# datatypevoid/babble

Measured on AMD Instinct MI355X. Metric: consensus-ordered events/sec at N=256 peers (1 GPU and 8-GPU batched sims), higher is better.
Workload: dtype int32

## Files before the change

babble_amd/csrc/hgx_api.cpp:

```cpp
#include <algorithm>
#include <array>
#include <chrono>
#include <cstdio>
#include <cstring>
#include <mutex>
#include <tuple>
#include <set>
#include <new>
#include <cstdlib>
#include <string>
#include <thread>
#include <vector>

#include "hgx.h"
#include "hgx_bodies.h"
#include "hgx_bodystore.h"
#include "hgx_diff.h"
#include "hgx_engine.h"
#include "hgx_wire_plan.h"

namespace {

struct Block {
    int32_t rr;
// ... 2736 lines not shown
    DeviceGuard dg(c);
    if (ensure_mirror(c) || !same_graph(c, x, y)) return 0;
    std::vector<int32_t> lx(c->n), fx(c->n), ly(c->n), fy(c->n);
    if (c->eng.get_coords(x, lx.data(), fx.data()) != hipSuccess) return 0;
    if (c->eng.get_coords(y, ly.data(), fy.data()) != hipSuccess) return 0;
    int cnt = 0;
    for (int i = 0; i < c->n; i++) cnt += lx[i] >= fy[i];
    return cnt >= c->sm ? 1 : 0;
}
int64_t hgx_oldest_self_ancestor_to_see(hgx_ctx* c, int64_t x, int64_t y) {
    if (!known_div(c, x) || !known_div(c, y)) return -1;
    DeviceGuard dg(c);
    if (ensure_chains(c) || !same_graph(c, x, y)) return -1;
    std::vector<int32_t> la(c->n), fd(c->n);
    if (c->eng.get_coords(y, la.data(), fd.data()) != hipSuccess) return -1;
    const int cx = c->creator[(size_t)x];
    const int32_t a = fd[cx % c->n];
    if (a <= c->index32[(size_t)x]) return c->chain_gids[cx][(size_t)(a - c->chain_base[cx])];
    return -1;
}
int32_t hgx_round(hgx_ctx* c, int64_t x) {
    if (!c) return -1;
    DeviceGuard dg(c);
    if (ensure_rounds(c)) return -1;
    return round_of(c, x);
}
int32_t hgx_witness(hgx_ctx* c, int64_t x) {
    if (!c) return 0;
    DeviceGuard dg(c);
    if (ensure_rounds(c) || ensure_mirror(c)) return 0;
    return witness_of(c, x);
}

int32_t hgx_phase_times(hgx_ctx* c, double* out, int32_t cap) {
    if (!c || !out) return 0;
    const int32_t m = std::min<int32_t>(cap, 28);
    double v[28] = {c->eng.phase_ms[0], c->eng.phase_ms[1], c->eng.phase_ms[2], c->eng.phase_ms[3],
                    (double)c->eng.la_sweeps, (double)c->eng.R, (double)c->eng.compact,
                    (double)c->eng.la_rows, c->eng.last_rebuild ? 1.0 : 0.0, (double)c->rh.r_lo,
                    c->eng.la_wave_used ? 1.0 : 0.0, (double)c->eng.la_wave_fallbacks,
                    (double)(c->eng.la_wave_used ? c->eng.la_wave_segs : 0), (double)c->eng.round_p_runs,
                    (double)c->eng.round_p_fallbacks, (double)c->eng.round_p_ovf,
                    (double)c->eng.round_p_fail_round, (double)c->eng.round_p_fail_chain,
                    (double)c->eng.round_g_runs, c->eng.la_small_used ? 1.0 : 0.0,
                    c->eng.la_verified ? 1.0 : 0.0, (double)c->eng.sort_seg_runs, (double)c->eng.pipe_used,
                    c->host_ms[0], c->host_ms[1], c->host_ms[2], c->host_ms[3], (double)c->eng.cts_row_runs};
    for (int32_t i = 0; i < m; i++) out[i] = v[i];
    return m;
}

static const char* kKernelNames[hgx::K_NUM] = {"layout", "la_sweep", "fd_build", "round_gather", "round_search",
                                              "fame", "threshold", "round_received", "cts_median", "order_sort"};

int32_t hgx_kernel_stats(hgx_ctx* c, int32_t k, char* name, int32_t name_cap, double* ms, int64_t* launches,
                         double* bytes) {
    if (!c || k < 0 || k >= hgx::K_NUM) return HGX_ERR_INVALID;
    if (name && name_cap > 0) std::snprintf(name, (size_t)name_cap, "%s", kKernelNames[k]);
    const hgx::KernelStat& ks = c->eng.kstat[k];
    if (ms) *ms = (ks.timed > 0 && ks.timed < ks.launches) ? ks.ms * (double)ks.launches / (double)ks.timed : ks.ms;
    if (launches) *launches = c->eng.kstat[k].launches;
    if (bytes) *bytes = c->eng.kstat[k].bytes;
    return HGX_OK;
}

int32_t hgx_reset_stats(hgx_ctx* c) {
    if (!c) return HGX_ERR_INVALID;
    for (auto& s : c->eng.kstat) s = hgx::KernelStat();
    return HGX_OK;
}

int32_t hgx_set_coord_storage(hgx_ctx* c, int32_t mode) {
    if (!c || mode < 0 || mode > 1) return HGX_ERR_INVALID;
    each_shard(c, [&](hgx_ctx* x) { x->eng.force_coord32 = mode == 1; });
    return HGX_OK;
}

int32_t hgx_set_kernel_timing(hgx_ctx* c, int32_t on) {
    if (!c) return HGX_ERR_INVALID;
    each_shard(c, [&](hgx_ctx* x) { x->eng.time_mask = (uint32_t)on; });
    return HGX_OK;
}

int32_t hgx_set_fame_tally(hgx_ctx* c, int32_t mode) {
    if (!c || mode < 0 || mode > 2) return HGX_ERR_INVALID;
    each_shard(c, [&](hgx_ctx* x) { x->eng.fame_tally = mode; });
    return HGX_OK;
}

int32_t hgx_device_alloc(int32_t device, int64_t bytes, void** ptr) {
    if (!ptr || bytes < 0) return HGX_ERR_INVALID;
    *ptr = nullptr;
    int prev = -1;
    (void)hipGetDevice(&prev);
    if (hipSetDevice(device) != hipSuccess) return HGX_ERR_DEVICE;
    const hipError_t e = hipMalloc(ptr, (size_t)std::max<int64_t>(bytes, 1));
    if (prev >= 0 && prev != device) (void)hipSetDevice(prev);
    return e == hipSuccess ? HGX_OK : HGX_ERR_DEVICE;
}

int32_t hgx_device_free(int32_t device, void* ptr) {
    int prev = -1;
    (void)hipGetDevice(&prev);
    if (hipSetDevice(device) != hipSuccess) return HGX_ERR_DEVICE;
    const hipError_t e = ptr ? hipFree(ptr) : hipSuccess;
    if (prev >= 0 && prev != device) (void)hipSetDevice(prev);
    return e == hipSuccess ? HGX_OK : HGX_ERR_DEVICE;
}

int32_t hgx_device_copy(int32_t device, void* dst, const void* src, int64_t bytes, int32_t to_device) {
    if (bytes < 0 || (bytes > 0 && (!dst || !src))) return HGX_ERR_INVALID;
    int prev = -1;
    (void)hipGetDevice(&prev);
    if (hipSetDevice(device) != hipSuccess) return HGX_ERR_DEVICE;
    const hipError_t e = bytes ? hipMemcpy(dst, src, (size_t)bytes, to_device ? hipMemcpyHostToDevice
                                                                               : hipMemcpyDeviceToHost)
                               : hipSuccess;
    if (prev >= 0 && prev != device) (void)hipSetDevice(prev);
    return e == hipSuccess ? HGX_OK : HGX_ERR_DEVICE;
}

int32_t hgx_set_ingest_pipeline(hgx_ctx* c, int32_t pieces, int64_t min_events) {
    if (!c || pieces < 0 || pieces > hgx::kPipeMaxPieces || min_events < 0) return HGX_ERR_INVALID;
    each_shard(c, [&](hgx_ctx* x) {
        x->eng.pipe_pieces = pieces;
        x->eng.pipe_min = min_events;
    });
    return HGX_OK;
}

int32_t hgx_set_la_kernel(hgx_ctx* c, int32_t mode) {
    if (!c || mode < 0 || mode > 1026) return HGX_ERR_INVALID;
    each_shard(c, [&](hgx_ctx* x) {
        x->eng.la_kernel = mode == 1 ? 1 : 0;
        x->eng.la_segs_override = (mode >= 2 && mode <= 1024) ? mode : 0;
        x->eng.la_small_override = mode == 1025 ? 0 : -1;
        x->eng.la_verify_always = mode == 1026;
    });
    return HGX_OK;
}

int32_t hgx_set_root_others(hgx_ctx* c, const uint8_t* event_hash32, int64_t count, hgx_error* err) {
    if (!c || count < 0 || (count > 0 && !event_hash32)) {
        set_err(err, HGX_ERR_INVALID, "hgx_set_root_others: bad arguments");
        return HGX_ERR_INVALID;
    }
    if (group_only_one(c, err, "hgx_set_root_others")) return HGX_ERR_INVALID;
    if (!c->rooted && count > 0) {
        set_err(err, HGX_ERR_INVALID, "hgx_set_root_others: no roots installed (hgx_reset)");
        return HGX_ERR_INVALID;
    }
    DeviceGuard dg(c);
    const hipError_t e = c->eng.set_root_others(event_hash32, count);
    if (e != hipSuccess) return dev_err(err, e, "hgx_set_root_others");
    c->others_keys.assign(event_hash32, event_hash32 + (size_t)count * 32);
    return ok(err);
}

int32_t hgx_set_sort_kernel(hgx_ctx* c, int32_t mode) {
    if (!c || mode < 0 || mode > 1) return HGX_ERR_INVALID;
    each_shard(c, [&](hgx_ctx* x) { x->eng.sort_seg_enabled = mode == 0; });
    return HGX_OK;
}

int32_t hgx_set_round_kernel(hgx_ctx* c, int32_t mode) {
    if (!c || mode < 0 || mode > 5) return HGX_ERR_INVALID;
    each_shard(c, [&](hgx_ctx* x) {
        x->eng.round_kernel = mode == 5 ? 0 : mode;
// ... 160 lines not shown
```

babble_amd/csrc/hgx_engine.cpp:

```cpp
#include "hgx_engine.h"
#include "hgx_bodystore.h"

#include <algorithm>
#include <array>
#include <chrono>
#include <cstdio>
#include <cstdlib>
#include <cstring>
#include <functional>

namespace hgx {

template <typename T>
hipError_t DBuf<T>::alloc(size_t count) {
    release();
    if (count == 0) count = 1;
    hipError_t e = hipMalloc((void**)&p, count * sizeof(T));
    if (e == hipSuccess) n = count; else p = nullptr;
    return e;
}

template <typename T>
hipError_t DBuf<T>::grow_copy(size_t count, size_t keep, hipStream_t s) {
    if (count <= n) return hipSuccess;
// ... 1291 lines not shown
    return hipStreamSynchronize(stream);
}

hipError_t Engine::get_event_fields(int64_t gid, int64_t* ts, int32_t* ntx, int32_t* tx_nil) {
    uint8_t nil = 0;
    HGX_TRY(hipMemcpyAsync(ts, g_ts.p + gid, 8, hipMemcpyDeviceToHost, stream));
    HGX_TRY(hipMemcpyAsync(ntx, g_ntx.p + gid, 4, hipMemcpyDeviceToHost, stream));
    HGX_TRY(hipMemcpyAsync(&nil, g_txnil.p + gid, 1, hipMemcpyDeviceToHost, stream));
    HGX_TRY(hipStreamSynchronize(stream));
    *tx_nil = nil;
    return hipSuccess;
}

hipError_t Engine::reserve_rounds(int32_t rounds) {
    rounds = std::max<int32_t>(rounds, 1);
    drop_step_graph();
    Bm.release(); WLA.release(); WFD.release(); wflag.release(); wstat.release(); wcoin.release();
    active.release(); Tthr.release(); fw.release(); elig.release(); ur_empty.release(); Smat.release();
    Vbuf.release(); fame.release(); blk_cnt.release(); blk_loaded.release(); blk_ntx.release(); blk_nil.release();
    ovf.release();
    WLAT.release();
    r_cap = 0;
    R = 0;
    E_div = 0;
    HGX_TRY(ensure_round_cap(rounds));
    return hipStreamSynchronize(stream);
}

int Engine::rebuild_segments(int64_t En, int coord_compact) const {
    if (G != 1 || En < (int64_t)kLaSegMinRows * C) return 1;
    const int cap_segs = (int)std::max<int64_t>(kLaMaxSegs, En / C / (2 * kLaHeadRows));
    return la_segs_override > 0 ? la_segs_override : la_wave_segments(n, coord_compact, num_cus, cap_segs);
}

void Engine::divide_rounds_rows(RoundsHost& out) {
    if (!rows_pending) return;
    rows_pending = false;
    for (size_t k = 0; k < rows_n && k < stage_out.size(); k++) {
        StagedD2H& d = stage_out[k];
        std::memcpy(d.dst, h_stage + d.off, d.bytes);
        d.bytes = 0;
    }
    out.bm.resize((size_t)(R + 1) * C);
    out.wflag.resize((size_t)R * C);
}

int32_t Engine::recv_round_lo(const RoundsHost& rh, int& max_unrecv) const {
    int32_t lo = R;
    max_unrecv = 0;
    if (E_div == 0 || rh.R == 0) return lo;
    for (int c = 0; c < C; c++) {
        const int32_t k = h_fu[c], len = h_len_div[c];
        if (k >= len) continue;
        max_unrecv = std::max(max_unrecv, len - k);
        int32_t a = 0, b = rh.R;
        while (a < b) {
            const int32_t mid = (a + b + 1) / 2;
            if (rh.bm[(size_t)mid * C + c] <= k) a = mid; else b = mid - 1;
        }
        lo = std::min(lo, a + 1);
    }
    return lo;
}

hipError_t Engine::decide_fame(int32_t r0, std::vector<int8_t>& fame_out) {
    HGX_TRY(decide_fame_launch(r0, fame_out));
    return fame_pending ? decide_fame_wait() : hipSuccess;
}

hipError_t Engine::decide_fame_launch(int32_t r0, std::vector<int8_t>& fame_out) {
    fame_pending = false;
    if (!rows_pending) {
        stage_out.clear();
        stage_used = 0;
    }
    pend.clear();
    if (fame_out.size() < (size_t)R * C) fame_out.resize((size_t)R * C, 0);
    r0 = std::max(r0, 0);
    if (R <= r0) return hipSuccess;
    DevArrays a = arrays();
    HGX_TRY(hipEventRecord(ph0, stream));
    HGX_TRY(hipGetLastError());
    kbeg(K_FAME);
    launch_fame(stream, a, r0, R, C, n, nw, sm, G, fame_tally);
    kend(K_FAME, 0);
    HGX_TRY(hipGetLastError());
    const size_t o = (size_t)r0 * C;
    HGX_TRY(stage_d2h(fame_out.data() + o, fame.p + o, fame_out.size() - o));
    HGX_TRY(stage_issue());
    HGX_TRY(hipEventRecord(ph1, stream));
    fame_pending = true;
    return hipSuccess;
}

hipError_t Engine::decide_fame_wait() {
    if (!fame_pending) {
        return hipStreamSynchronize(stream);
    }
    fame_pending = false;
    HGX_TRY(hipEventSynchronize(ph1));
    stage_flush();
    float ms = 0;
    HGX_TRY(hipEventElapsedTime(&ms, ph0, ph1));
    phase_ms[2] = ms;
    return collect_kernel_times();
}

hipError_t Engine::find_order(const std::vector<uint8_t>& el, const std::vector<uint8_t>& famous,
                              const std::vector<uint8_t>& ure, int32_t r0, int max_unrecv, OrderHost& out) {
    HGX_TRY(find_order_begin(el, famous, ure, r0, max_unrecv, out));
    return find_order_end(out, nullptr);
}

hipError_t Engine::find_order_begin(const std::vector<uint8_t>& el, const std::vector<uint8_t>& famous,
                                    const std::vector<uint8_t>& ure, int32_t r0, int max_unrecv, OrderHost& out) {
    stage_out.clear();
    pend.clear();
    stage_used = 0;
    out = OrderHost();
    fo_m = 0;
    fo_cnt.assign(C, 0);
    if (R == 0 || E_div == 0 || max_unrecv == 0 || r0 >= R) return hipSuccess;
    DevArrays a = arrays();
    HGX_TRY(hipEventRecord(ph0, stream));
    const size_t o = (size_t)r0 * C;
    HGX_TRY(stage_h2d(elig.p, el.data(), (size_t)G * R));
    HGX_TRY(stage_h2d(fw.p + o, famous.data() + o, (size_t)R * C - o));
    HGX_TRY(stage_h2d(ur_empty.p, ure.data(), (size_t)G));
    HGX_TRY(stage_issue());
    if (WLAT.n < (size_t)R * C * n) {
        const size_t want = (size_t)R * C * n + (size_t)C * n;
        const size_t first = WLAT.n ? 0 : std::min((size_t)r_cap * C * n, (size_t)1 << 28);
        HGX_TRY(WLAT.alloc(std::max(want, std::max(2 * WLAT.n, first))));
        a = arrays();
    }
    kbeg(K_THRESHOLD);
    launch_wla_transpose(stream, a, r0, R, G, C, n);
    launch_threshold(stream, a, r0, R, C, n);
    kend(K_THRESHOLD, 0);
    {
        FillRange fr[2] = {{counters.p + kCtRecv, 8, 0}, {rcnt.p, (uint32_t)((size_t)C * 4), 0}};
        launch_fill_many(stream, fr, 2);
        HGX_TRY(hipGetLastError());
    }
    kbeg(K_ROUND_RECEIVED);
    launch_round_received(stream, a, R, C, n, max_unrecv);
    kend(K_ROUND_RECEIVED, 0);
    HGX_TRY(copy_to_pinned(h_small + kHsRecv, counters.p + kCtRecv, 8));
    HGX_TRY(stage_d2h(fo_cnt.data(), rcnt.p, (size_t)C * 4));
    HGX_TRY(stage_issue());
    HGX_TRY(hipStreamSynchronize(stream));
    stage_flush();
    fo_m = h_small[kHsRecv];
    out.panic = h_small[kHsRecv + 1] != 0;
    out.m = fo_m;
    int max_cnt = 0, unrecv = 0;
    for (int c = 0; c < C; c++) unrecv += h_len_div[c] - h_fu[c];
    for (int c = shard_lo; c < shard_hi; c++) max_cnt = std::max(max_cnt, fo_cnt[c]);
    kadd_bytes(K_ROUND_RECEIVED, (double)unrecv * 16);
    if (out.panic || fo_m == 0) {
        fo_m = 0;
        return collect_kernel_times();
    }
    int64_t own = 0;
    for (int c = shard_lo; c < shard_hi; c++) own += fo_cnt[c];
    const int c_cnt = shard_hi - shard_lo;
    constexpr int kCtsRowMinTiles = 8;
// ... 259 lines not shown
```

babble_amd/csrc/hgx_kernels.h:

```cpp
#pragma once

#include <hip/hip_runtime.h>

#include <cstdint>
#include <functional>
#include <vector>

namespace hgx {

constexpr int32_t kMaxI32 = 2147483647;
constexpr int32_t kWlatNotFamous = -2147483647 - 1;
constexpr int kOpkBits = 21;

struct DevArrays {
    const int32_t *g_creator, *g_index, *g_op, *g_ntx;
    const int64_t* g_ts;
    const uint8_t *g_S, *g_coin, *g_loaded, *g_txnil;
    int32_t *g_rr, *g_pos;
    int64_t* g_ck;
    int64_t* g_cts;
    const int32_t *c_off, *c_len, *c_base;
    int32_t *p_gid, *p_chain, *p_op, *p_opu, *p_round, *p_rr;
    int32_t* p_opk;
    int64_t *p_ts, *p_cts;
// ... 84 lines not shown
hipError_t ensure_lds_limit(const void* f, size_t bytes);
hipError_t blocks_per_cu(const void* f, int T, size_t lds, int* out);

struct FillRange {
    void* p;
    uint32_t bytes;
    uint8_t value;
};
constexpr int kFillMax = 8;
void launch_fill_many(hipStream_t s, const FillRange* r, int count);
struct CopyRange {
    const void* src;
    void* dst;
    uint32_t bytes;
    int reset = -1;
};
constexpr int kCopyMax = 8;
void launch_copy_many(hipStream_t s, const CopyRange* r, int count);

int fd_tile_rows(int n, int compact);
void launch_layout(hipStream_t s, int64_t E0, int64_t E, const DevArrays& a, int C, int n, int seg,
                   const int32_t* gate = nullptr);
bool la_wave_ok(int n, int max_len, int n_active);
size_t la_small_bytes(int n, int compact, int64_t P);
hipError_t launch_la_small(hipStream_t s, const DevArrays& a, int G, int n, const int32_t* c_old, size_t lds,
                           int32_t* err);
int la_wave_blocks(int n, int compact);
int la_wave_segments(int n, int compact, int num_cus, int max_segs);
hipError_t launch_la_seg_check(hipStream_t s, const DevArrays& a, int n, int64_t E, int nts, int head, int32_t* tbl,
                               int32_t* flag);
struct LaSubset {
    int first = 0, count = 0;
    const int32_t* c_lim = nullptr;
    const int32_t* gate = nullptr;
};
hipError_t launch_la_wave(hipStream_t s, const DevArrays& a, int G, int n, const int32_t* c_old, int64_t E, int nts,
                          int head, int32_t* err, const int32_t* lmap = nullptr, int na = 0,
                          bool narrow = false, const LaSubset& sub = LaSubset());
void launch_la_sweep(hipStream_t s, const DevArrays& a, int C, int n, int max_len, int seg, int first, int32_t* chg,
                     int32_t stamp, int64_t* usum, int32_t* out, int32_t* out_next, const int32_t* c_old, int64_t u0);
void launch_fd_build(hipStream_t s, const DevArrays& a, int C, int n, int max_len, int64_t P, const int32_t* c_old,
                     int max_new, int d_lo = 0, int d_hi = -1);
void launch_init_new(hipStream_t s, const DevArrays& a, int64_t E0, int64_t m, int n, int64_t P);
void launch_round_gather(hipStream_t s, const DevArrays& a, int r, int C, int n, int64_t P);
void launch_wcoin(hipStream_t s, const DevArrays& a, int r0, int R, int C);
hipError_t launch_round_step(hipStream_t s, const RoundArgs& A, int r, int block_search);
hipError_t launch_round_k(hipStream_t s, const RoundArgs& A, int r);
void launch_round_k_gather(hipStream_t s, const RoundArgs& A, int r);
int round_k_ndw(int n);
bool round_p_ok(int n, int C, int num_cus);
bool round_g_ok(int n, int nw);
hipError_t launch_round_g(hipStream_t s, const RoundArgs& A, int32_t* status, int32_t* fin, int r0, int r_end);
constexpr int kRoundPBufs = 4;
constexpr int kRoundPShift = 2;
constexpr int kMaxShards = 8;
struct RoundPWindows {
    int nwin = 0;
    uint32_t remote = 0;
    uint32_t* FD8p[kMaxShards] = {};
    uint64_t* gran[kMaxShards] = {};
    int32_t* st[kMaxShards] = {};
    const void* FDT[kMaxShards] = {};
    int32_t c_split[kMaxShards + 1] = {};
};
hipError_t launch_xchg_floor(hipStream_t s, int C, int n, int rounds, uint32_t* rows, uint64_t* gran, int32_t* st);
hipError_t launch_round_p(hipStream_t s, const RoundArgs& A, uint32_t* FD8p, uint64_t* gran, int32_t* status,
                          int32_t* fin, int r0, int r_end, int init, int num_cus, int c_lo = 0, int c_hi = -1,
                          const RoundPWindows* win_dev = nullptr, int nwin = 1);
void launch_round_p_tail(hipStream_t s, const RoundArgs& A, const int32_t* fin, int r_last);
void launch_round_p_post(hipStream_t s, const RoundArgs& A, int r_lo, int r_hi);
bool round_pb_ok(int n, int G);
hipError_t launch_round_pb(hipStream_t s, const RoundArgs& A, uint32_t* FD8p, uint64_t* gran, int32_t* status,
                           int32_t* fin, const int32_t* amap, int na, int r0, int r_end, int num_cus, bool init);
void launch_round_pb_silent(hipStream_t s, const RoundArgs& A, int r_lo, int r_hi);
void launch_root_floor(hipStream_t s, const DevArrays& a, const int32_t* root_round, int32_t* gfl, int32_t* gB,
                       int gmax, int C, int n, int max_len);
void launch_round_first_gid(hipStream_t s, const DevArrays& a, int r0, int R, int C, int32_t* first);
void launch_last_round(hipStream_t s, int rs, int R, int G, int C, int n, const uint8_t* wstat, int32_t* lr);
void step_prof_dump();
void round_k_prof_dump();
void round_p_prof_dump();
void round_pb_prof_dump();
void round_g_prof_dump();
void launch_fame(hipStream_t s, const DevArrays& a, int r0, int R, int C, int n, int nw, int sm, int G, int tally);
void launch_wla_transpose(hipStream_t s, const DevArrays& a, int r0, int R, int G, int C, int n);
void launch_threshold(hipStream_t s, const DevArrays& a, int r0, int R, int C, int n);
void launch_round_received(hipStream_t s, const DevArrays& a, int R, int C, int n, int max_unrecv);
void launch_fu_advance(hipStream_t s, const DevArrays& a, int C);
void launch_fu_count(hipStream_t s, const DevArrays& a, int64_t E);
void launch_cts(hipStream_t s, const DevArrays& a, int c_lo, int c_cnt, int C, int n, int64_t P, int max_cnt);
bool cts_pipe_ok(int n, int C);
bool launch_cts_pipe(hipStream_t s, const DevArrays& a, int c_lo, int c_cnt, int C, int n, int64_t P, int max_cnt);
bool cts_row_ok(int n);
int cts_row_tile();
bool launch_cts_row(hipStream_t s, const DevArrays& a, int c_lo, int c_cnt, int C, int n, int64_t P, int max_cnt,
                    int R, int k_rows);
void launch_cts_shard_copy(hipStream_t s, const DevArrays& a, int lo, int hi, const int32_t* offs, int64_t* buf,
                           int to_buf);
void launch_minmax(hipStream_t s, const DevArrays& a, int32_t m);
void launch_sort(hipStream_t s, const DevArrays& a, int32_t m, int64_t cmin, int cts_bits, int R, int n,
                 int seg_bits, uint32_t** final_vals, uint64_t** final_keys);
int seg_sort_cap();
void launch_seg_count(hipStream_t s, const DevArrays& a, int32_t m, int R, int n, int nseg, uint32_t* segc,
                      unsigned long long* max_out);
hipError_t launch_sort_seg(hipStream_t s, const DevArrays& a, int32_t m, int64_t cmin, int cts_bits, int R, int n, int nseg,
                     uint32_t* segoff, uint32_t* segcur, int max_seg, uint32_t** final_vals, uint64_t** final_keys,
                     const std::vector<int>* cuts = nullptr,
                     const std::function<hipError_t(int)>& after_part = nullptr);
bool sort_small_ok(int32_t m);
void launch_sort_small(hipStream_t s, const DevArrays& a, int32_t m, int n, uint32_t** final_vals);
void launch_finish_order(hipStream_t s, const DevArrays& a, int32_t m, const uint32_t* vals, int R, int n);
void launch_gather_i32(hipStream_t s, int64_t E, const int32_t* src, const int32_t* g_pos, int32_t* dst);

size_t p256_table_bytes(int nk);
void launch_p256_tables(hipStream_t s, int nk, const uint8_t* keys65, uint32_t* tab, uint8_t* valid);
void launch_p256_verify(hipStream_t s, int64_t count, int nk, const int32_t* key_idx, const uint8_t* dig,
                        const uint8_t* r, const uint8_t* sg, const uint32_t* tab, const uint8_t* valid, uint8_t* out);
constexpr int kSignBlock = 64;
constexpr size_t kP256TabWords = (size_t)32 * 256 * 16;
void launch_p256_sign(hipStream_t s, int64_t count, const int32_t* key_idx, const uint8_t* priv32, const uint8_t* dig,
                      const uint32_t* tab_g, uint8_t* out_r, uint8_t* out_s);
void launch_p256_pub(hipStream_t s, int nk, const uint8_t* priv32, const uint32_t* tab_g, uint8_t* out65);
bool p256_scalar_ok(const uint8_t* d32);

void launch_insert_claim(hipStream_t s, int64_t m, int64_t E0, int64_t cap, int C, const InsertIn& in,
                         const InsertState& st);
void launch_insert_check(hipStream_t s, int64_t m, int64_t E0, int64_t cap, int C, int n, const InsertIn& in,
                         const InsertState& st);
constexpr int kCommitAll = 0, kCommitStructure = 1, kCommitPayload = 2;
void launch_insert_commit(hipStream_t s, int64_t m, const unsigned long long* fail, const unsigned long long* fail_sig,
                          int64_t E0, int n, const InsertIn& in, const InsertState& st, int mode);
constexpr int kPipeMaxPieces = 8;
void launch_pipe_hist(hipStream_t s, int pieces, const int64_t* cut, int C, const int32_t* creator, int32_t* hist);
void launch_pipe_insert(hipStream_t s, int64_t m, int64_t E0, int64_t cap, int C, int n, const InsertIn& in,
                        const InsertState& st, int32_t* gate);
void launch_ts_to_pos(hipStream_t s, int64_t E0, int64_t m, const int32_t* g_pos, const int64_t* g_ts, int64_t* p_ts);
void launch_insert_unclaim(hipStream_t s, int64_t m, const unsigned long long* fail, const unsigned long long* fail_sig,
                           int64_t E0, int64_t cap, int C, const InsertIn& in, const InsertState& st);
bool launch_insert_fused(hipStream_t s, int64_t m, const unsigned long long* fail_sig, int64_t E0, int64_t cap, int C,
                         int n, const InsertIn& in, const InsertState& st, int mode);
void launch_insert_sig_first(hipStream_t s, int64_t m, int C, const int32_t* creator, const uint8_t* vout,
                             unsigned long long* fail);
void launch_unpack_packed(hipStream_t s, int64_t m, int64_t E0, const uint16_t* c16, const uint16_t* spb,
                          const uint16_t* opb, int64_t n_exc, const int64_t* exc_pos, const int32_t* exc_sp,
                          const int32_t* exc_op, int32_t* cr, int32_t* sp, int32_t* op);

void launch_scan_u32(hipStream_t s, uint32_t* buf, int64_t total, uint32_t* part);

struct PruneArgs {
    int64_t E, n_kept;
    int C;
    const int32_t *g_creator, *g_index, *g_sp, *g_op, *g_ntx;
    const int64_t* g_ts;
    const uint8_t *g_S, *g_id, *g_txnil;
    const int32_t* cut;
    uint32_t* scan;
    int32_t* first_gid;
    uint32_t* kept_total;
    int32_t *st_creator, *st_index, *st_sp, *st_op, *st_ntx, *old_gid;
    int64_t* st_ts;
    uint8_t *st_hash, *st_S;
    uint32_t* oth_count;
    int32_t *oth_new, *oth_op;
    uint8_t *oth_key, *oth_pid;
    int32_t *root_sp, *root_op;
    uint8_t* root_ids;
};
// ... 36 lines not shown
```

babble_amd/csrc/hgx_kernels.hip:

```cpp
#include <hip/hip_runtime.h>

#include <algorithm>
#include <cstdint>
#include <cstdlib>
#include <cstring>
#include <map>
#include <mutex>
#include <tuple>

#include "hgx.h"
#include "hgx_device.h"
#include "hgx_kernels.h"

namespace hgx {


constexpr int kLayoutB = 4096;
constexpr int kLayoutH = 1024;

__global__ void __launch_bounds__(256) k_ck_pack(int64_t E0, int64_t E, const int32_t* __restrict__ g_creator,
                                                 const int32_t* __restrict__ g_index, const int32_t* __restrict__ c_base,
                                                 int64_t* __restrict__ g_ck, const int32_t* __restrict__ gate) {
    if (gate && *gate) return;
    const int64_t gid = E0 + (int64_t)blockIdx.x * blockDim.x + threadIdx.x;
// ... 770 lines not shown
            }
        }
        __syncthreads();
        auto vote = [&](int yi, int x, int yays) {
            const int y = ys[yi];
            const int nays = ytot[yi] - yays;
            const bool v = yays >= nays;
            const int tt = v ? yays : nays;
            bool bit;
            if (normal) {
                if (tt >= sm) atomicCAS(&dec[x], 0, v ? 1 : 2);
                bit = v;
            } else {
                bit = (tt >= sm) ? v : (wcoin[jr + y] != 0);
            }
            if (bit) atomicOr((unsigned long long*)&Vb[cur ^ 1][x][y >> 6], 1ull << (y & 63));
        };
        if constexpr (kMfma) {
            const int h = lane >> 4, r16 = lane & 15;
            const signed char* img = reinterpret_cast<const signed char*>(fsm);
            for (int rp = wave; rp * 32 < ny; rp += 4) {
                int4v acc[2][4];
#pragma unroll
                for (int a = 0; a < 2; a++)
#pragma unroll
                    for (int b = 0; b < 4; b++) acc[a][b] = int4v{0, 0, 0, 0};
                const int yi0 = rp * 32 + r16, yi1 = yi0 + 16;
                const uint64_t* s0 = yi0 < ny ? Smat + (jr + ys[yi0]) * nw : nullptr;
                const uint64_t* s1 = yi1 < ny ? Smat + (jr + ys[yi1]) * nw : nullptr;
                for (int k = 0; k < nw; k++) {
                    const uint64_t w0 = s0 ? (s0[k] & wm[k]) : 0ull;
                    const uint64_t w1 = s1 ? (s1[k] & wm[k]) : 0ull;
                    const int4v a0 = expand16((uint32_t)(w0 >> (16 * h)) & 0xFFFFu);
                    const int4v a1 = expand16((uint32_t)(w1 >> (16 * h)) & 0xFFFFu);
#pragma unroll
                    for (int b = 0; b < 4; b++) {
                        const int4v bf = *reinterpret_cast<const int4v*>(img + (b * 16 + r16) * KB + k * 64 + 16 * h);
                        acc[0][b] = __builtin_amdgcn_mfma_i32_16x16x64_i8(a0, bf, acc[0][b], 0, 0, 0);
                        acc[1][b] = __builtin_amdgcn_mfma_i32_16x16x64_i8(a1, bf, acc[1][b], 0, 0, 0);
                    }
                }
#pragma unroll
                for (int a = 0; a < 2; a++)
#pragma unroll
                    for (int b = 0; b < 4; b++)
#pragma unroll
                        for (int q = 0; q < 4; q++) {
                            const int yi = rp * 32 + a * 16 + 4 * h + q, x = b * 16 + r16;
                            if (yi < ny && x < nxt) vote(yi, x, acc[a][b][q]);
                        }
            }
        } else {
            const int x = lane;
            uint64_t vx[kFameMaxW];
#pragma unroll
            for (int k = 0; k < kFameMaxW; k++) vx[k] = k < nw ? Vb[cur][x][k] : 0ull;
            for (int yi = wave; yi < ny; yi += 4) {
                int yays = 0;
                if (s_lds) {
                    const uint64_t* srow = sS + yi * nw;
#pragma unroll
                    for (int k = 0; k < kFameMaxW; k++)
                        if (k < nw) yays += __popcll(srow[k] & vx[k]);
                } else {
                    const uint64_t* srow = Smat + (jr + ys[yi]) * nw;
#pragma unroll
                    for (int k = 0; k < kFameMaxW; k++)
                        if (k < nw) yays += __popcll(srow[k] & wm[k] & vx[k]);
                }
                if (x < nxt) vote(yi, x, yays);
            }
        }
        __syncthreads();
        if (threadIdx.x < 64) {
            const bool u = (int)threadIdx.x < nxt && dec[threadIdx.x] == 0;
            const uint64_t m = __ballot(u);
            if (threadIdx.x == 0) s_und = __popcll(m);
        }
        __syncthreads();
        if (s_und == 0) break;
        cur ^= 1;
    }
    if ((int)threadIdx.x < nxt) fame[(size_t)i * C + gi + xs[threadIdx.x]] = (int8_t)dec[threadIdx.x];
}

__global__ void __launch_bounds__(256) k_wla_transpose(int R, int r0, int G, int C, int n,
                                                       const uint8_t* __restrict__ elig, const uint8_t* __restrict__ fw,
                                                       const int32_t* __restrict__ WLA, int32_t* __restrict__ WLAT) {
    __shared__ int32_t t[64][65];
    const int ig = blockIdx.y, i = r0 + ig / G, g = ig % G;
    if (!elig[(size_t)g * R + i]) return;
    const int nt = (n + 63) / 64, tc = blockIdx.x % nt, td = blockIdx.x / nt;
    const size_t base = ((size_t)i * C + (size_t)g * n) * n;
    if ((n & 63) == 0) {
        const uint8_t* __restrict__ fwr = fw + (size_t)i * C + (size_t)g * n + tc * 64;
        const int c4 = (threadIdx.x & 15) * 4, r4 = threadIdx.x >> 4;
#pragma unroll
        for (int h = 0; h < 4; h++) {
            const int r = r4 + 16 * h;
            const int4 v = *(const int4*)(WLA + base + (size_t)(tc * 64 + r) * n + td * 64 + c4);
            const bool f = fwr[r] != 0;
            t[r][c4] = f ? v.x : kWlatNotFamous;
            t[r][c4 + 1] = f ? v.y : kWlatNotFamous;
            t[r][c4 + 2] = f ? v.z : kWlatNotFamous;
            t[r][c4 + 3] = f ? v.w : kWlatNotFamous;
        }
        __syncthreads();
#pragma unroll
        for (int h = 0; h < 4; h++) {
            const int d = r4 + 16 * h;
            *(int4*)(WLAT + base + (size_t)(td * 64 + d) * n + tc * 64 + c4) =
                make_int4(t[c4][d], t[c4 + 1][d], t[c4 + 2][d], t[c4 + 3][d]);
        }
        return;
    }
    for (int k = threadIdx.x; k < 64 * 64; k += 256) {
        const int r = k >> 6, col = k & 63, c = tc * 64 + r, d = td * 64 + col;
        t[r][col] = (c < n && d < n) ? (fw[(size_t)i * C + (size_t)g * n + c] ? WLA[base + (size_t)c * n + d]
                                                                               : kWlatNotFamous) : 0;
    }
    __syncthreads();
    for (int k = threadIdx.x; k < 64 * 64; k += 256) {
        const int r = k >> 6, col = k & 63, d = td * 64 + r, c = tc * 64 + col;
        if (c < n && d < n) WLAT[base + (size_t)d * n + c] = t[col][r];
    }
}

template <int CPL>
__global__ void __launch_bounds__(256) k_threshold(int R, int r0, const uint8_t* __restrict__ elig,
                            const uint8_t* __restrict__ fw,
                            const int32_t* __restrict__ WLAT, int32_t* __restrict__ T, int C, int n) {
    const int64_t item = ((int64_t)blockIdx.x * blockDim.x + threadIdx.x) >> 6;
    if (item >= (int64_t)(R - r0) * C) return;
    const int i = r0 + (int)(item / C), gd = (int)(item % C);
    const int g = gd / n;
    if (!elig[(size_t)g * R + i]) return;
    const int lane = lane_id();
    const size_t row = ((size_t)i * C + gd) * n;
    uint32_t v[CPL];
    bool ok[CPL];
    int m = 0;
#pragma unroll
    for (int q = 0; q < CPL; q++) {
        const int c = lane + 64 * q;
        const int32_t x = c < n ? WLAT[row + c] : kWlatNotFamous;
        ok[q] = x != kWlatNotFamous;
        v[q] = (uint32_t)x ^ 0x80000000u;
        m += __popcll(__ballot(ok[q]));
    }
    int32_t res = -1;
    if (m > 0) {
        const uint32_t u = wave_select_kth32_bisect<CPL>(v, ok, m - 1 - m / 2);
        res = (int32_t)(u ^ 0x80000000u);
    }
    if (lane == 0) T[(size_t)i * C + gd] = res;
}

constexpr int kRrPer = 4;
__global__ void __launch_bounds__(256) k_round_received(int R, const int32_t* __restrict__ c_off,
                                 const int32_t* __restrict__ c_len, const int32_t* __restrict__ c_base,
                                 const int32_t* __restrict__ fu, const int32_t* __restrict__ p_round,
                                 const int32_t* __restrict__ lr, const uint8_t* __restrict__ elig,
                                 const uint8_t* __restrict__ ur_empty, const int32_t* __restrict__ T,
                                 int32_t* __restrict__ p_rr, int32_t* __restrict__ rcnt, int32_t* __restrict__ recv_list,
                                 int32_t* __restrict__ counters, int C, int n) {
    __shared__ int32_t s_wcnt[kRrPer][4], s_base;
// ... 1140 lines not shown
                       a.p_opu, a.p_opk, a.p_ts, a.p_rr, a.p_cts, C, n, seg, gate);
}

void launch_la_sweep(hipStream_t s, const DevArrays& a, int C, int n, int max_len, int seg, int first, int32_t* chg,
                     int32_t stamp, int64_t* usum, int32_t* out, int32_t* out_next, const int32_t* c_old, int64_t u0) {
    const int nseg = (max_len + seg - 1) / seg;
    if ((int64_t)nseg * C <= u0) return;
    const int nwd = a.compact ? n / 2 : n;
#define LA_LAUNCH_V(GS, CPL, CT, V)                                                                           \
    {                                                                                                         \
        const int64_t threads = ((int64_t)nseg * C - u0) * GS;                                                \
        hipLaunchKernelGGL((k_la_sweep<GS, CPL, CT, V>), dim3(std::min(nblk(threads, 256), 2048u)), dim3(256), 0, \
                           s, (uint32_t*)a.LA, a.p_op, a.p_opu, a.c_off, a.c_len, a.c_base, C, n, nwd, nseg, seg, \
                           first ? 1 : 0, chg, stamp, usum, out, out_next, c_old, u0);                        \
    }
#define LA_LAUNCH_T(GS, CPL, CT)                                   \
    {                                                              \
        if (first == 2) LA_LAUNCH_V(GS, CPL, CT, true) else LA_LAUNCH_V(GS, CPL, CT, false) \
    }
#define LA_LAUNCH(GS, CPL, NW)                                        \
    {                                                                 \
        if (a.compact) LA_LAUNCH_T(GS, CPL, uint16_t) else LA_LAUNCH_T(GS, CPL, int32_t) \
    }
    HGX_DISPATCH_N(nwd, LA_LAUNCH);
#undef LA_LAUNCH
#undef LA_LAUNCH_T
#undef LA_LAUNCH_V
}

int fd_tile_rows(int n, int compact) {
    (void)compact;
    return n <= 32 ? 256 : 128;
}

int fd_cols(int compact, int ft) { return (compact ? 256 : 128) * 64 / ft; }

void launch_fd_build(hipStream_t s, const DevArrays& a, int C, int n, int max_len, int64_t P, const int32_t* c_old,
                     int max_new, int d_lo, int d_hi) {
    if (d_hi < 0) d_hi = n;
    if (d_hi <= d_lo) return;
    const int ft = fd_tile_rows(n, a.compact);
    const int tiles = c_old ? max(1, (max_new + ft - 1) / ft) : max(1, (max_len + ft - 1) / ft);
    const int nwd = a.compact ? n / 2 : n;
    const int DB = std::min(fd_cols(a.compact, ft), d_hi - d_lo);
    const int ncb = (d_hi - d_lo + DB - 1) / DB;
    const int wdw = DB / (a.compact ? 2 : 1) + 1;
    const size_t lds = ((size_t)(ft + 1) * (wdw + 1) + 1 + 3 * (size_t)DB + 8 * 128) * sizeof(int32_t);
    const int zs = (c_old && max_new <= ft) ? max(1, min(8, DB / 64)) : 1;
    const dim3 grid(C, tiles, ncb * zs);
#define FD_LAUNCH(CT_, RPL_)                                                                                    \
    hipLaunchKernelGGL((k_fd_build<CT_, RPL_>), grid, dim3(512), lds, s, (const uint32_t*)a.LA, (CT_*)a.FDT, a.c_off, \
                       a.c_len, a.c_base, n, nwd, ft, P, c_old, d_lo, d_hi, DB, zs)
    if (a.compact) {
        if (ft == 256) FD_LAUNCH(uint16_t, 4);
        else if (ft == 128) FD_LAUNCH(uint16_t, 2);
        else FD_LAUNCH(uint16_t, 1);
    } else {
        if (ft == 256) FD_LAUNCH(int32_t, 4);
        else if (ft == 128) FD_LAUNCH(int32_t, 2);
        else FD_LAUNCH(int32_t, 1);
    }
#undef FD_LAUNCH
}

void launch_round_gather(hipStream_t s, const DevArrays& a, int r, int C, int n, int64_t P) {
    if (a.compact)
        hipLaunchKernelGGL(k_round_gather<uint16_t>, dim3(nblk((int64_t)C * n, 256)), dim3(256), 0, s, r, a.Bm,
                           a.c_off, a.c_len, (const uint16_t*)a.LA, (const uint16_t*)a.FDT, a.p_gid, a.g_coin, a.WLA,
                           a.WFD, a.wflag, a.wcoin, C, n, P, 1);
    else
        hipLaunchKernelGGL(k_round_gather<int32_t>, dim3(nblk((int64_t)C * n, 256)), dim3(256), 0, s, r, a.Bm,
                           a.c_off, a.c_len, (const int32_t*)a.LA, (const int32_t*)a.FDT, a.p_gid, a.g_coin, a.WLA,
                           a.WFD, a.wflag, a.wcoin, C, n, P, 0);
}

void launch_wcoin(hipStream_t s, const DevArrays& a, int r0, int R, int C) {
    const int64_t RC = (int64_t)(R - r0) * C;
    if (RC <= 0) return;
    const size_t o = (size_t)r0 * C;
    hipLaunchKernelGGL(k_wcoin, dim3(nblk(RC, 256)), dim3(256), 0, s, RC, C, a.Bm + o, a.c_off, a.c_len, a.p_gid,
                       a.g_coin, a.wcoin + o);
}

void launch_fame(hipStream_t s, const DevArrays& a, int r0, int R, int C, int n, int nw, int sm, int G, int tally) {
    if (R <= r0) return;
    const int mode = tally == 1 ? 0 : tally == 2 ? 2 : 1;
    if (mode != 0 && n <= kFameMaxW * 64) {
        const int XT = (n + kFameTile - 1) / kFameTile;
        const dim3 grid((unsigned)((int64_t)G * (R - r0) * XT));
        if (mode == 2) {
            const int shm = kFameTile * (nw * 64 + 16);
            (void)ensure_lds_limit((const void*)k_fame_tile<true>, kFameTile * (kFameMaxW * 64 + 16));
            hipLaunchKernelGGL(k_fame_tile<true>, grid, dim3(256), shm, s, R, r0, XT, a.lr, a.wstat, a.wcoin, a.Bm,
                               a.c_base, a.WLA, a.Smat, a.fame, C, n, nw, sm, 0);
        } else {
            const int sw = (size_t)n * nw * 8 <= kFameSW * 8 ? n * nw : 0;
            hipLaunchKernelGGL(k_fame_tile<false>, grid, dim3(256), (size_t)sw * 8, s, R, r0, XT, a.lr, a.wstat, a.wcoin,
                               a.Bm, a.c_base, a.WLA, a.Smat, a.fame, C, n, nw, sm, sw);
        }
        return;
    }
    hipLaunchKernelGGL(k_fame_vote, dim3((unsigned)G * (R - r0)), dim3(256), 0, s, R, r0, nw, a.lr, a.wstat, a.wcoin, a.Bm,
                       a.c_base, a.WLA, a.Smat, a.Vbuf, a.fame, C, n, sm);
}

void launch_wla_transpose(hipStream_t s, const DevArrays& a, int r0, int R, int G, int C, int n) {
    if (R <= r0) return;
    const int nt = (n + 63) / 64;
    hipLaunchKernelGGL(k_wla_transpose, dim3(nt * nt, (R - r0) * G), dim3(256), 0, s, R, r0, G, C, n, a.elig, a.fw, a.WLA,
                       a.WLAT);
}

void launch_threshold(hipStream_t s, const DevArrays& a, int r0, int R, int C, int n) {
    if (R <= r0) return;
#define TH_LAUNCH(GS, CPL, NW)                                                                                \
    {                                                                                                         \
        const int64_t threads = (int64_t)(R - r0) * C * 64;                                                   \
        hipLaunchKernelGGL((k_threshold<CPL>), dim3(nblk(threads, 256)), dim3(256), 0, s, R, r0, a.elig, a.fw, \
                           a.WLAT, a.T, C, n);                                                                \
    }
    HGX_DISPATCH_N(n, TH_LAUNCH);
#undef TH_LAUNCH
}

void launch_round_received(hipStream_t s, const DevArrays& a, int R, int C, int n, int max_unrecv) {
    if (max_unrecv <= 0) return;
    hipLaunchKernelGGL(k_round_received, dim3(nblk(max_unrecv, 256 * kRrPer), C), dim3(256), 0, s, R, a.c_off, a.c_len,
                       a.c_base, a.fu, a.p_round, a.lr, a.elig, a.ur_empty, a.T, a.p_rr, a.rcnt, a.recv_list,
                       a.counters, C, n);
}

void launch_fu_advance(hipStream_t s, const DevArrays& a, int C) {
    hipLaunchKernelGGL(k_fu_advance, dim3(nblk(C, 256)), dim3(256), 0, s, C, a.fu, a.rcnt);
}

void launch_fu_count(hipStream_t s, const DevArrays& a, int64_t E) {
    if (E > 0) hipLaunchKernelGGL(k_fu_count, dim3(nblk(E, 256)), dim3(256), 0, s, E, a.g_creator, a.g_rr, a.fu);
}

void launch_init_new(hipStream_t s, const DevArrays& a, int64_t E0, int64_t m, int n, int64_t P) {
    if (m <= 0) return;
    if (a.compact)
        hipLaunchKernelGGL(k_init_new<uint16_t>, dim3(nblk(m, 16), (n + 63) / 64), dim3(256), 0, s, E0, m, a.g_pos,
                           (uint16_t*)a.LA, (uint16_t*)a.FDT, n, P);
    else
        hipLaunchKernelGGL(k_init_new<int32_t>, dim3(nblk(m, 16), (n + 63) / 64), dim3(256), 0, s, E0, m, a.g_pos,
                           (int32_t*)a.LA, (int32_t*)a.FDT, n, P);
}

template <int NP, typename CT>
static void cts_small_launch(hipStream_t s, const DevArrays& a, int c_lo, int c_cnt, int C, int n, int64_t P,
                             int max_cnt) {
    hipLaunchKernelGGL((k_cts_small<NP, CT>), dim3(nblk(max_cnt, 256), c_cnt), dim3(256), 0, s, a.fu, a.rcnt, a.p_rr,
                       a.c_off, a.c_base, a.fw, a.WLAT, (const CT*)a.FDT, a.p_ts, a.p_cts, C, n, P, c_lo);
}

template <int NPAD, typename CT>
static void cts_tile_launch(hipStream_t s, const DevArrays& a, int c_lo, int c_cnt, int C, int n, int64_t P,
                            int max_cnt) {
    const size_t lds = (size_t)NPAD * (kCtsTile + 1) * sizeof(uint32_t);
    (void)ensure_lds_limit((const void*)k_cts_tile<NPAD, CT>, lds);
    const int64_t ntiles = (max_cnt + kCtsTile - 1) / kCtsTile;
    const int64_t g64 = (int64_t)64 * ((c_cnt + 7) / 8) * ((ntiles + 7) / 8);
    if (g64 == 0) return;
    hipLaunchKernelGGL((k_cts_tile<NPAD, CT>), dim3((unsigned)g64), dim3(256), lds, s, a.fu, a.rcnt, a.p_rr,
                       a.c_off, a.c_base, a.fw, a.WLAT, (const CT*)a.FDT, a.p_ts, a.p_cts, C, n, P, c_lo, c_cnt);
}

// ... 331 lines not shown
```

babble_amd/hashgraph.py:

```python
from __future__ import annotations

import ctypes as C
import os
from typing import List, Optional, Sequence

import numpy as np

from . import _lib
from ._lib import HgxError, hgx_error, hgx_events, ptr

UNKNOWN_PARENT = -2


def compact_columns(t) -> dict:
    ntx = np.where(np.asarray(t.txnil) != 0, -1, np.asarray(t.ntx)).astype(np.int32)
    return dict(creator=np.ascontiguousarray(t.creator, np.int32), index=np.ascontiguousarray(t.index, np.int32),
                sp=np.ascontiguousarray(t.sp, np.int32), op=np.ascontiguousarray(t.op, np.int32),
                ts=np.ascontiguousarray(t.ts, np.int64),
                coin=np.ascontiguousarray(np.asarray(t.hash)[:, 16] != 0, np.uint8),
                s=np.ascontiguousarray(t.s, np.uint8), ntx=ntx)


class HostBuffer:

# ... 758 lines not shown
        return res

    def Ancestor(self, x: int, y: int) -> bool:
        return bool(self.L.hgx_ancestor(self.ctx, x, y))

    def SelfAncestor(self, x: int, y: int) -> bool:
        return bool(self.L.hgx_self_ancestor(self.ctx, x, y))

    def See(self, x: int, y: int) -> bool:
        return bool(self.L.hgx_see(self.ctx, x, y))

    def StronglySee(self, x: int, y: int) -> bool:
        return bool(self.L.hgx_strongly_see(self.ctx, x, y))

    def OldestSelfAncestorToSee(self, x: int, y: int) -> int:
        return int(self.L.hgx_oldest_self_ancestor_to_see(self.ctx, x, y))

    def Round(self, x: int) -> int:
        return int(self.L.hgx_round(self.ctx, x))

    def Witness(self, x: int) -> bool:
        return bool(self.L.hgx_witness(self.ctx, x))

    def coords(self, x: int):
        la = np.zeros(self.n, np.int32)
        fd = np.zeros(self.n, np.int32)
        rc = self.L.hgx_get_coords(self.ctx, x, ptr(la), ptr(fd))
        if rc:
            raise HgxError(rc, "hgx_get_coords failed")
        return la, fd

    def num_events(self) -> int:
        return int(self.L.hgx_num_events(self.ctx))

    def rounds(self):
        E = self.num_events()
        rnd = np.zeros(max(E, 1), np.int32)
        wit = np.zeros(max(E, 1), np.int8)
        fam = np.zeros(max(E, 1), np.int8)
        if E:
            rc = self.L.hgx_get_rounds(self.ctx, 0, E, ptr(rnd), ptr(wit), ptr(fam))
            if rc:
                raise HgxError(rc, "hgx_get_rounds failed")
        return rnd[:E], wit[:E], fam[:E]

    def received(self):
        E = self.num_events()
        rr = np.zeros(max(E, 1), np.int32)
        cts = np.zeros(max(E, 1), np.int64)
        if E:
            rc = self.L.hgx_get_received(self.ctx, 0, E, ptr(rr), ptr(cts))
            if rc:
                raise HgxError(rc, "hgx_get_received failed")
        return rr[:E], cts[:E]

    def results(self, graph: int = 0) -> dict:
        rnd, wit, fam = self.rounds()
        rr, cts = self.received()
        return dict(round=rnd, witness=wit, famous=fam, rr=rr, cts=np.where(rr >= 0, cts, 0),
                    order=self.ConsensusEvents(graph), last_round=self.LastRound(graph),
                    undecided=self.UndecidedRounds(graph), lcr=self.LastConsensusRound(graph),
                    lcre=self.LastCommitedRoundEvents(graph), consensus_tx=self.ConsensusTransactions(graph),
                    pending_loaded=self.PendingLoadedEvents(graph), blocks=self.Blocks(graph))

    def phase_times(self):
        out = np.zeros(28, np.float64)
        self.L.hgx_phase_times(self.ctx, ptr(out), 28)
        return dict(coords_ms=out[0], rounds_ms=out[1], fame_ms=out[2], order_ms=out[3],
                    la_sweeps=int(out[4]), rounds=int(out[5]), compact=int(out[6]),
                    la_rows=int(out[7]), rebuild=int(out[8]), r_lo=int(out[9]),
                    la_wave=int(out[10]), la_wave_fallbacks=int(out[11]), la_wave_segs=int(out[12]),
                    round_p_runs=int(out[13]), round_p_fallbacks=int(out[14]), round_p_ovf=int(out[15]),
                    round_p_fail_round=int(out[16]), round_p_fail_chain=int(out[17]),
                    round_g_runs=int(out[18]), la_small=int(out[19]), la_verify=int(out[20]),
                    sort_seg=int(out[21]), ingest_pieces=int(out[22]),
                    host_rounds_ms=out[23], host_fame_ms=out[24], host_order_ms=out[25],
                    payload_end_ms=out[26], cts_row=int(out[27]))

    def set_ingest_pipeline(self, pieces, min_events=4_000_000):
        if self.L.hgx_set_ingest_pipeline(self.ctx, int(pieces), int(min_events)) != 0:
            raise ValueError(f"invalid ingest pipeline {pieces}, {min_events}")

    def set_fame_tally(self, mode):
        m = {"popc": 0, "vote": 1, "mfma": 2}[mode] if isinstance(mode, str) else int(mode)
        if self.L.hgx_set_fame_tally(self.ctx, m) != 0:
            raise ValueError(f"invalid fame tally {mode}")

    def set_la_kernel(self, mode):
        m = {"wave": 0, "sweep": 1, "ring": 1025, "wave+verify": 1026}[mode] if isinstance(mode, str) else int(mode)
        if self.L.hgx_set_la_kernel(self.ctx, m) != 0:
            raise ValueError(f"invalid lastAncestors kernel {mode}")

    def set_round_kernel(self, mode):
        m = ({"auto": 0, "block": 1, "candidate": 2, "persistent": 3, "graph": 4, "auto-steps": 5}[mode]
             if isinstance(mode, str) else int(mode))
        if self.L.hgx_set_round_kernel(self.ctx, m) != 0:
            raise ValueError(f"invalid round kernel {mode}")

    def set_sort_kernel(self, mode):
        m = {"auto": 0, "radix": 1}[mode] if isinstance(mode, str) else int(mode)
        if self.L.hgx_set_sort_kernel(self.ctx, m) != 0:
            raise ValueError(f"invalid sort kernel {mode}")

    def set_round_shards(self, shards: int):
        if self.L.hgx_set_round_shards(self.ctx, int(shards)) != 0:
            raise ValueError(f"invalid shard count {shards} (an empty context, 1..8 shards, "
                             f"GPU_MAX_HW_QUEUES >= shards + 2 for shards sharing a device)")

    def set_shard_remote(self, on: bool = True):
        if self.L.hgx_set_shard_remote(self.ctx, 1 if on else 0) != 0:
            raise ValueError("hgx_set_shard_remote: not a chain-sharded context")

    def set_cts_kernel(self, mode):
        m = {"auto": 0, "tile": 1, "pipe": 2, "row": 3, "row1": 4}[mode] if isinstance(mode, str) else int(mode)
        if self.L.hgx_set_cts_kernel(self.ctx, m) != 0:
            raise ValueError(f"invalid timestamp kernel {mode}")

    def set_incremental(self, on: bool):
        if self.L.hgx_set_incremental(self.ctx, 1 if on else 0) != 0:
            raise ValueError("invalid schedule")

    def reserve_rounds(self, rounds: int):
        if self.L.hgx_reserve_rounds(self.ctx, int(rounds)) != 0:
            raise ValueError("hgx_reserve_rounds failed")

    def set_coord_storage(self, mode):
        if self.L.hgx_set_coord_storage(self.ctx, int(mode)) != 0:
            raise ValueError(f"invalid coordinate storage mode {mode}")

    def kernel_stats(self):
        res = {}
        for k in range(10):
            name = C.create_string_buffer(32)
            ms, launches, nbytes = C.c_double(), C.c_int64(), C.c_double()
            if self.L.hgx_kernel_stats(self.ctx, k, name, 32, C.byref(ms), C.byref(launches), C.byref(nbytes)):
                break
            res[name.value.decode()] = dict(ms=ms.value, launches=launches.value, bytes=nbytes.value)
        return res

    KERNELS = ("layout", "la_sweep", "fd_build", "round_gather", "round_search", "fame", "threshold",
               "round_received", "cts_median", "order_sort")

    def set_kernel_timing(self, which=True):
        if which is True:
            mask = -1
        elif not which:
            mask = 0
        else:
            mask = 1 << self.KERNELS.index(which)
        self.L.hgx_set_kernel_timing(self.ctx, mask)

    def reset_stats(self):
        self.L.hgx_reset_stats(self.ctx)


class DeviceBuffer:

    def __init__(self, a: np.ndarray, device: int = 0):
        self.L = _lib.lib()
        self.device = device
        a = np.ascontiguousarray(a)
        self.nbytes = a.nbytes
        self.p = C.c_void_p()
        if self.L.hgx_device_alloc(device, max(1, a.nbytes), C.byref(self.p)) != 0:
            raise HgxError(200, "hgx_device_alloc failed")
        if a.nbytes and self.L.hgx_device_copy(device, self.p, ptr(a), a.nbytes, 1) != 0:
            self.close()
# ... 190 lines not shown
```

Baseline: 288.0 million.

## Add wavefront-per-voter fame kernel with adaptive witness slicing for popc tally

Adds a new fame-decision kernel in which each wavefront handles 64 voters and a block covers a slice of candidate witnesses. Vote bitmasks are kept in shared memory and double-buffered across rounds, and tallies are done with popcount over the strongly-seen masks. The slice width is chosen from the CU count so the grid holds enough blocks. This becomes the default path when tally mode is 0 and n fits, replacing the previous tile/vote kernels there. The old default behaviour moves to a new mode 3 ('tile'). The aim is better parallelism and data reuse in fame voting, at the cost of recomputing the first-round votes in each slice block.

```diff
diff --git a/babble_amd/csrc/hgx_api.cpp b/babble_amd/csrc/hgx_api.cpp
--- a/babble_amd/csrc/hgx_api.cpp
+++ b/babble_amd/csrc/hgx_api.cpp
@@ -2842,7 +2842,7 @@
 }
 
 int32_t hgx_set_fame_tally(hgx_ctx* c, int32_t mode) {
-    if (!c || mode < 0 || mode > 2) return HGX_ERR_INVALID;
+    if (!c || mode < 0 || mode > 3) return HGX_ERR_INVALID;
     each_shard(c, [&](hgx_ctx* x) { x->eng.fame_tally = mode; });
     return HGX_OK;
 }
diff --git a/babble_amd/csrc/hgx_engine.cpp b/babble_amd/csrc/hgx_engine.cpp
--- a/babble_amd/csrc/hgx_engine.cpp
+++ b/babble_amd/csrc/hgx_engine.cpp
@@ -1397,7 +1397,7 @@
     HGX_TRY(hipEventRecord(ph0, stream));
     HGX_TRY(hipGetLastError());
     kbeg(K_FAME);
-    launch_fame(stream, a, r0, R, C, n, nw, sm, G, fame_tally);
+    launch_fame(stream, a, r0, R, C, n, nw, sm, G, fame_tally, num_cus);
     kend(K_FAME, 0);
     HGX_TRY(hipGetLastError());
     const size_t o = (size_t)r0 * C;
diff --git a/babble_amd/csrc/hgx_kernels.h b/babble_amd/csrc/hgx_kernels.h
--- a/babble_amd/csrc/hgx_kernels.h
+++ b/babble_amd/csrc/hgx_kernels.h
@@ -190,7 +190,8 @@
 void round_p_prof_dump();
 void round_pb_prof_dump();
 void round_g_prof_dump();
-void launch_fame(hipStream_t s, const DevArrays& a, int r0, int R, int C, int n, int nw, int sm, int G, int tally);
+void launch_fame(hipStream_t s, const DevArrays& a, int r0, int R, int C, int n, int nw, int sm, int G, int tally,
+                 int num_cus);
 void launch_wla_transpose(hipStream_t s, const DevArrays& a, int r0, int R, int G, int C, int n);
 void launch_threshold(hipStream_t s, const DevArrays& a, int r0, int R, int C, int n);
 void launch_round_received(hipStream_t s, const DevArrays& a, int R, int C, int n, int max_unrecv);
diff --git a/babble_amd/csrc/hgx_kernels.hip b/babble_amd/csrc/hgx_kernels.hip
--- a/babble_amd/csrc/hgx_kernels.hip
+++ b/babble_amd/csrc/hgx_kernels.hip
@@ -876,6 +876,131 @@
         cur ^= 1;
     }
     if ((int)threadIdx.x < nxt) fame[(size_t)i * C + gi + xs[threadIdx.x]] = (int8_t)dec[threadIdx.x];
+}
+
+constexpr int kFameSlice = 64;
+
+template <int NW>
+__global__ void __launch_bounds__(64 * NW) k_fame_voter(int R, int r0, int XT, int XS, const int32_t* __restrict__ lr,
+                            const uint8_t* __restrict__ wstat, const uint8_t* __restrict__ wcoin,
+                            const int32_t* __restrict__ Bm, const int32_t* __restrict__ c_base,
+                            const int32_t* __restrict__ WLA, const uint64_t* __restrict__ Smat,
+                            int8_t* __restrict__ fame, int C, int n, int sm) {
+    __shared__ uint64_t V[2][kFameSlice][NW];
+    __shared__ uint64_t wm[2][NW];
+    __shared__ int8_t decw[2][NW][kFameSlice];
+    const int RR = R - r0;
+    const int xt = blockIdx.x % XT;
+    const int i = r0 + (blockIdx.x / XT) % RR;
+    const int g = blockIdx.x / (XT * RR);
+    const int LR = lr[g];
+    if (i > LR) return;
+    const size_t gi = (size_t)g * n;
+    const int lane = lane_id();
+    const int q = __builtin_amdgcn_readfirstlane((int)(threadIdx.x >> 6));
+    const int y = 64 * q + lane;
+    const bool yin = y < n;
+    const int yc = yin ? y : 0;
+    const int x0 = xt * XS;
+    const int nxs = min(XS, n - x0);
+    const size_t xr = (size_t)i * C + gi + x0;
+    const bool isx = lane < nxs && wstat[xr + (lane < nxs ? lane : 0)] == 2;
+    const uint64_t xmask = __ballot(isx);
+    if (xmask == 0) return;
+    if (i + 2 > LR) {
+        if (q == 0 && isx) fame[xr + lane] = 0;
+        return;
+    }
+    {
+        const size_t jr = (size_t)(i + 1) * C + gi;
+        const bool act = yin && wstat[jr + yc] == 2;
+        const uint64_t am = __ballot(act);
+        if (lane == 0) wm[(i + 1) & 1][q] = am;
+        const int32_t xi = isx ? c_base[gi + x0 + lane] + Bm[xr + lane] : 0x7FFFFFFF;
+        const int32_t* __restrict__ row = WLA + (jr + yc) * n + x0;
+        uint64_t nv = 0;
+        for (int xb = 0; xb < nxs; xb += 8) {
+            int32_t la[8];
+#pragma unroll
+            for (int u = 0; u < 8; u++) la[u] = row[min(xb + u, nxs - 1)];
+#pragma unroll
+            for (int u = 0; u < 8; u++) {
+                const uint64_t b = __ballot(la[u] >= __builtin_amdgcn_readlane(xi, xb + u)) & am;
+                if (lane == xb + u) nv = b;
+            }
+        }
+        V[0][lane][q] = nv;
+    }
+    __syncthreads();
+    int dec = 0;
+    int cur = 0;
+    for (int j = i + 2; j <= LR; j++) {
+        const bool normal = ((j - i) % n) != 0;
+        const size_t jr = (size_t)j * C + gi;
+        const bool act = yin && wstat[jr + yc] == 2;
+        const uint64_t am = __ballot(act);
+        if (lane == 0) wm[j & 1][q] = am;
+        const bool coin = wcoin[jr + yc] != 0;
+        const uint64_t* __restrict__ srow = Smat + (jr + yc) * NW;
+        const uint64_t* wp = wm[(j - 1) & 1];
+        uint64_t S[NW];
+        int tot = 0;
+#pragma unroll
+        for (int k = 0; k < NW; k++) S[k] = srow[k];
+#pragma unroll
+        for (int k = 0; k < NW; k++) {
+            S[k] = act ? S[k] & wp[k] : 0ull;
+            tot += __popcll(S[k]);
+        }
+        uint64_t nv = 0;
+        int nd = 0;
+        auto vote = [&](int xl, const uint64_t* vx) {
+            int yays = 0;
+#pragma unroll
+            for (int k = 0; k < NW; k++) yays += __popcll(S[k] & vx[k]);
+            const int nays = tot - yays;
+            const bool v = yays >= nays;
+            const bool strong = (v ? yays : nays) >= sm;
+            uint64_t bits;
+            if (normal) {
+                const uint64_t vb = __ballot(v);
+                const uint64_t d = __ballot(strong) & am;
+                const int val = d ? 2 - (int)((vb >> __builtin_ctzll(d)) & 1ull) : 0;
+                if (lane == xl) nd = val;
+                bits = vb & am;
+            } else {
+                bits = __ballot(strong ? v : coin) & am;
+            }
+            if (lane == xl) nv = bits;
+        };
+        for (uint64_t rem = xmask & __ballot(dec == 0); rem;) {
+            const int xa = __builtin_ctzll(rem);
+            rem &= rem - 1;
+            const int xb = rem ? __builtin_ctzll(rem) : xa;
+            rem &= rem - 1;
+            uint64_t va[NW], vb[NW];
+#pragma unroll
+            for (int k = 0; k < NW; k++) {
+                va[k] = V[cur][xa][k];
+                vb[k] = V[cur][xb][k];
+            }
+            vote(xa, va);
+            vote(xb, vb);
+        }
+        V[cur ^ 1][lane][q] = nv;
+        if (normal) decw[j & 1][q][lane] = (int8_t)nd;
+        __syncthreads();
+        if (normal) {
+#pragma unroll
+            for (int k = 0; k < NW; k++) {
+                const int d = decw[j & 1][k][lane];
+                dec = dec ? dec : d;
+            }
+        }
+        if ((xmask & __ballot(dec == 0)) == 0) break;
+        cur ^= 1;
+    }
+    if (q == 0 && isx) fame[xr + lane] = (int8_t)dec;
 }
 
 __global__ void __launch_bounds__(256) k_wla_transpose(int R, int r0, int G, int C, int n,
@@ -2182,8 +2307,33 @@
                        a.g_coin, a.wcoin + o);
 }
 
-void launch_fame(hipStream_t s, const DevArrays& a, int r0, int R, int C, int n, int nw, int sm, int G, int tally) {
+static int fame_slice(int n, int nw, int64_t graph_rounds, int num_cus) {
+    const int64_t slots = (int64_t)num_cus * std::max(1, std::min(8, 32 / nw));
+    int xs = kFameSlice;
+    while (xs > 16 && graph_rounds * ((n + xs - 1) / xs) < 2 * slots) xs >>= 1;
+    return xs;
+}
+
+void launch_fame(hipStream_t s, const DevArrays& a, int r0, int R, int C, int n, int nw, int sm, int G, int tally,
+                 int num_cus) {
     if (R <= r0) return;
+    if (tally == 0 && n <= kFameMaxW * 64) {
+        const int XS = fame_slice(n, nw, (int64_t)G * (R - r0), num_cus);
+        const int XT = (n + XS - 1) / XS;
+        const dim3 grid((unsigned)((int64_t)G * (R - r0) * XT));
+#define FV_LAUNCH(NW)                                                                                              \
+    case NW:                                                                                                       \
+        hipLaunchKernelGGL(k_fame_voter<NW>, grid, dim3(64 * NW), 0, s, R, r0, XT, XS, a.lr, a.wstat, a.wcoin, a.Bm, \
+                           a.c_base, a.WLA, a.Smat, a.fame, C, n, sm);                                             \
+        break;
+        switch (nw) {
+            FV_LAUNCH(1) FV_LAUNCH(2) FV_LAUNCH(3) FV_LAUNCH(4) FV_LAUNCH(5) FV_LAUNCH(6) FV_LAUNCH(7) FV_LAUNCH(8)
+            FV_LAUNCH(9) FV_LAUNCH(10) FV_LAUNCH(11) FV_LAUNCH(12) FV_LAUNCH(13) FV_LAUNCH(14) FV_LAUNCH(15)
+            FV_LAUNCH(16)
+        }
+#undef FV_LAUNCH
+        return;
+    }
     const int mode = tally == 1 ? 0 : tally == 2 ? 2 : 1;
     if (mode != 0 && n <= kFameMaxW * 64) {
         const int XT = (n + kFameTile - 1) / kFameTile;
diff --git a/babble_amd/hashgraph.py b/babble_amd/hashgraph.py
--- a/babble_amd/hashgraph.py
+++ b/babble_amd/hashgraph.py
@@ -864,7 +864,7 @@
             raise ValueError(f"invalid ingest pipeline {pieces}, {min_events}")
 
     def set_fame_tally(self, mode):
-        m = {"popc": 0, "vote": 1, "mfma": 2}[mode] if isinstance(mode, str) else int(mode)
+        m = {"popc": 0, "vote": 1, "mfma": 2, "tile": 3}[mode] if isinstance(mode, str) else int(mode)
         if self.L.hgx_set_fame_tally(self.ctx, m) != 0:
             raise ValueError(f"invalid fame tally {mode}")
 
```

Result: faster. 293.9 million (median of 6 runs) (+2.0%).
